# jewettaij/visfd

Measured on AMD Instinct MI355X. Metric: Mvoxels/s (Gauss+DoG+TV pipeline) on 1024^3 float32; % HBM roofline, higher is better.
Workload: dtype f32

## Files before the change

visfd_amd/csrc/blob.hip:

```cpp
#include <algorithm>
#include <cstdlib>
#include <limits>

#include "common.hpp"

namespace vh {

namespace {

constexpr int BLOCK = 512;
constexpr int TX = 64, TY = 8;
constexpr int PZ = 4;
constexpr int BUFCAP = 2 * PZ * BLOCK;
constexpr int LW = TX + 2, LH = TY + 2;

static_assert(BLOCK == 512 && TX == 64, "candidate codes pack the thread index in 9 bits");

struct Cand {
  int ix, iy, iz;
  int kind;
  float score;
};

__global__ void __launch_bounds__(BLOCK)
blob_candidates_kernel(const float* __restrict__ mid, const float* __restrict__ mask, int nx, int ny, int nz,
                       float min_thr, float max_thr, int zchunk, int tiles_x, int tiles_y,
                       unsigned long long* __restrict__ out, unsigned long long capacity,
                       unsigned long long* __restrict__ counter) {
  constexpr int NLD = (LH * LW + BLOCK - 1) / BLOCK;
  __shared__ float tile[PZ][NLD * BLOCK];
  __shared__ unsigned int buf[BUFCAP];
  __shared__ unsigned int buf_n;
  __shared__ unsigned long long buf_base;
  if (threadIdx.x == 0) buf_n = 0;
  unsigned b = blockIdx.x;
  const int tile_x = b % tiles_x;
  b /= tiles_x;
  const int tile_y = b % tiles_y;
  const int chunk = b / tiles_y;
  const int x0 = tile_x * TX, y0 = tile_y * TY;
  const int zs = max(1, chunk * zchunk), ze = min(nz - 1, (chunk + 1) * zchunk);
  if (zs >= ze) return;
  const int tid = threadIdx.x;
  const int lx = tid & (TX - 1), ly = tid >> 6;
  const int gx = x0 + lx, gy = y0 + ly;
  const i64 plane = (i64)nx * ny;
  const bool interior = gx >= 1 && gx <= nx - 2 && gy >= 1 && gy <= ny - 2;

  unsigned ld_off[NLD];
#pragma unroll
  for (int k = 0; k < NLD; k++) {
    const int i = tid + k * BLOCK;
    const int r = i / LW, c = i - r * LW;
    const int sx = x0 - 1 + c, sy = y0 - 1 + r;
    ld_off[k] = (i < LH * LW && sx >= 0 && sx < nx && sy >= 0 && sy < ny) ? (unsigned)(sy * nx + sx) * 4u : 0x7ffffff0u;
  }
  const int plane_bytes = (int)(plane * 4);
  auto fetch = [&](int z, float v[NLD]) {
    const bool zin = z < nz;
    const __amdgpu_buffer_rsrc_t rs = __builtin_amdgcn_make_buffer_rsrc((void*)(mid + (zin ? (i64)z * plane : 0)), 0,
                                                                        zin ? plane_bytes : 0, 0x00020000);
#pragma unroll
    for (int k = 0; k < NLD; k++) v[k] = __builtin_bit_cast(float, __builtin_amdgcn_raw_buffer_load_b32(rs, (int)ld_off[k], 0, 0));
  };
  auto stash = [&](const float v[NLD], float* dst) {
#pragma unroll
    for (int k = 0; k < NLD; k++) dst[tid + k * BLOCK] = v[k];
  };
  auto minmax9 = [&](const float* t, float& mn, float& mx, float& centre) {
    const float* p0 = t + ly * LW + lx;
    float a = p0[0], bb = p0[1], c = p0[2];
    mn = fminf(fminf(a, bb), c); mx = fmaxf(fmaxf(a, bb), c);
    a = p0[LW]; bb = p0[LW + 1]; c = p0[LW + 2];
    centre = bb;
    mn = fminf(mn, fminf(fminf(a, bb), c)); mx = fmaxf(mx, fmaxf(fmaxf(a, bb), c));
    a = p0[2 * LW]; bb = p0[2 * LW + 1]; c = p0[2 * LW + 2];
    mn = fminf(mn, fminf(fminf(a, bb), c)); mx = fmaxf(mx, fmaxf(fmaxf(a, bb), c));
  };

  float mn_prev, mx_prev, c_prev, mn_cur, mx_cur, c_cur;
  float preA[PZ][NLD], preB[PZ][NLD];
  fetch(zs - 1, preA[0]);
  fetch(zs, preA[1]);
  stash(preA[0], tile[0]);
  stash(preA[1], tile[1]);
#pragma unroll
  for (int k = 0; k < PZ; k++) fetch(zs + 1 + k, preA[k]);
#pragma unroll
  for (int k = 0; k < PZ; k++) fetch(zs + PZ + 1 + k, preB[k]);
  __syncthreads();
  minmax9(tile[0], mn_prev, mx_prev, c_prev);
  minmax9(tile[1], mn_cur, mx_cur, c_cur);
  __syncthreads();
  auto step = [&](float (&pre)[PZ][NLD], int z0) {
#pragma unroll
    for (int k = 0; k < PZ; k++) stash(pre[k], tile[k]);
#pragma unroll
    for (int k = 0; k < PZ; k++) fetch(z0 + 2 * PZ + 1 + k, pre[k]);
    __syncthreads();
#pragma unroll
    for (int k = 0; k < PZ; k++) {
      const int z = z0 + k;
      if (z < ze) {
        float mn_nxt, mx_nxt, c_nxt;
        minmax9(tile[k], mn_nxt, mx_nxt, c_nxt);
        const float e = c_cur;
        const float bmin = fminf(fminf(mn_prev, mn_cur), mn_nxt);
        const float bmax = fmaxf(fmaxf(mx_prev, mx_cur), mx_nxt);
        const bool is_min = (e == bmin) && (e < 0.0f) && (e < min_thr);
        const bool is_max = (e == bmax) && (e > 0.0f) && (e > max_thr);
        {
          const i64 v = (i64)z * plane + (i64)gy * nx + gx;
          bool cand = interior && (is_min || is_max);
          if (cand && mask && mask[v] == 0.0f) cand = false;
          const unsigned long long bal = __ballot(cand);
          if (bal != 0ull) {
            const int lane = tid & 63;
            const int leader = __ffsll((long long)bal) - 1;
            unsigned int base = 0;
            if (lane == leader) base = atomicAdd(&buf_n, (unsigned int)__popcll(bal));
            base = (unsigned int)__shfl((int)base, leader);
            if (cand) buf[base + (unsigned int)__popcll(bal & ((1ull << lane) - 1ull))] = ((unsigned int)(z - zs) << 9) | (unsigned int)tid;
          }
        }
        mn_prev = mn_cur; mx_prev = mx_cur;
        mn_cur = mn_nxt; mx_cur = mx_nxt; c_cur = c_nxt;
      }
    }
    __syncthreads();
    const unsigned int n = buf_n;
    const bool last = z0 + PZ >= ze;
    if (n > (unsigned int)(BUFCAP - PZ * BLOCK) || (last && n)) {
      if (tid == 0) buf_base = atomicAdd(counter, (unsigned long long)n);
      __syncthreads();
      const unsigned long long base = buf_base;
      for (unsigned int i = tid; i < n; i += BLOCK)
        if (base + i < capacity) {
          const unsigned int code = buf[i];
          const int t = (int)(code & 511u), zz = zs + (int)(code >> 9);
          out[base + i] = (unsigned long long)((i64)zz * plane + (i64)(y0 + (t >> 6)) * nx + (x0 + (t & (TX - 1))));
        }
      __syncthreads();
      if (tid == 0) buf_n = 0;
    }
  };
  for (int z0 = zs; z0 < ze; z0 += 2 * PZ) {
    step(preA, z0);
    step(preB, z0 + PZ);
  }
}

__global__ void __launch_bounds__(BLOCK)
blob_verify_kernel(const unsigned long long* __restrict__ cand_idx, const unsigned long long* __restrict__ n_cand_ptr,
                   unsigned long long cand_capacity,
                   const float* __restrict__ lo, const float* __restrict__ mid, const float* __restrict__ hi,
                   const float* __restrict__ mask, int nx, int ny, int nz, float min_thr, float max_thr,
                   Cand* __restrict__ out, unsigned long long capacity, unsigned long long* __restrict__ counter) {
  unsigned long long n_cand = *n_cand_ptr;
  if (n_cand > cand_capacity) n_cand = cand_capacity;
  for (unsigned long long t = (unsigned long long)blockIdx.x * BLOCK + threadIdx.x; t < n_cand;
       t += (unsigned long long)gridDim.x * BLOCK) {
  const i64 c = (i64)cand_idx[t];
  const i64 plane = (i64)nx * ny;
  const int iz = (int)(c / plane);
  const int rem = (int)(c - (i64)iz * plane);
  const int iy = rem / nx, ix = rem - iy * nx;
  const float e = mid[c];
  bool is_min = (e < 0.0f) && (e < min_thr);
  bool is_max = (e > 0.0f) && (e > max_thr);
  {
    const float a = lo[c], b = hi[c];
    if (a <= e || b <= e) is_min = false;
    if (a >= e || b >= e) is_max = false;
  }
  const float* vol[3] = {mid, lo, hi};
  for (int r = 0; r < 3 && (is_min || is_max); r++) {
    const float* v = vol[r];
    for (int jz = -1; jz <= 1; jz++)
      for (int jy = -1; jy <= 1; jy++) {
        const i64 row = c + (i64)jz * plane + (i64)jy * nx;
#pragma unroll
        for (int jx = -1; jx <= 1; jx++) {
          if (r == 0 && jz == 0 && jy == 0 && jx == 0) continue;
          const i64 q = row + jx;
          if (mask && r == 0 && mask[q] == 0.0f) { is_min = false; is_max = false; }
          const float nb = v[q];
          if (nb <= e) is_min = false;
          if (nb >= e) is_max = false;
        }
      }
  }
  if (is_min || is_max) {
    const unsigned long long slot = atomicAdd(counter, 1ULL);
    if (slot < capacity) {
      Cand cd;
      cd.ix = ix; cd.iy = iy; cd.iz = iz;
      cd.kind = is_min ? 0 : 1;
      cd.score = e;
      out[slot] = cd;
    }
  }
  }
}

}

struct ScanBufs {
  unsigned long long* idx = nullptr;
  Cand* cand = nullptr;
  unsigned long long* counters = nullptr;
  size_t cap_idx = 0, cap_out = 0;
};

static int scan_bufs(visfd_hip_ctx* ctx, int set, ScanBufs* B, bool pipelined, i64 nvox) {
  constexpr size_t NSET = 3;
  size_t cap_idx = ctx->slot_bytes[WS_TVAUX] / sizeof(unsigned long long) / NSET;
  if (cap_idx < (1u << 22)) cap_idx = 1u << 22;
  if (cap_idx < (size_t)(nvox / 32)) cap_idx = (size_t)(nvox / 32);
  size_t cap_out = ctx->slot_bytes[WS_CAND] / sizeof(Cand) / NSET;
  if (cap_out < (1u << 20)) cap_out = 1u << 20;
  if (cap_out < (size_t)(nvox / 128)) cap_out = (size_t)(nvox / 128);
  unsigned long long* idx = nullptr;
  Cand* cand = nullptr;
  unsigned long long* counters = nullptr;
  VH_TRY(ws(ctx, WS_TVAUX, NSET * cap_idx, &idx));
  VH_TRY(ws(ctx, WS_CAND, NSET * cap_out, &cand));
  VH_TRY(ws(ctx, WS_SCANCNT, 8, &counters));
  B->idx = idx + (size_t)set * cap_idx;
  B->cand = cand + (size_t)set * cap_out;
  B->counters = counters + 2 * set;
  B->cap_idx = cap_idx;
  B->cap_out = cap_out;
  if (pipelined) {
    if (ctx->opt.blob_test_cap > 0) {
      const size_t v = (size_t)ctx->opt.blob_test_cap;
      if (v < B->cap_idx) B->cap_idx = v;
      if (v < B->cap_out) B->cap_out = v;
    }
  }
  return VISFD_HIP_OK;
}

static void sort_and_append(std::vector<Cand>& h, i64 nx, i64 ny, int scale_index, float sigma,
                            std::vector<visfd_hip_blob>* minima, std::vector<visfd_hip_blob>* maxima) {
  const size_t m = h.size();
  std::vector<unsigned long long> key(m), key2(m);
  std::vector<unsigned int> pos(m), pos2(m);
  unsigned long long maxkey = 0;
  for (size_t i = 0; i < m; i++) {
    key[i] = (unsigned long long)(((i64)h[i].iz * ny + h[i].iy) * nx + h[i].ix);
    pos[i] = (unsigned int)i;
    if (key[i] > maxkey) maxkey = key[i];
  }
  constexpr int RB = 11;
  for (int shift = 0; shift < 64 && (maxkey >> shift) != 0; shift += RB) {
    size_t hist[(1 << RB) + 1] = {0};
    for (size_t i = 0; i < m; i++) hist[((key[i] >> shift) & ((1u << RB) - 1)) + 1]++;
    for (int b = 0; b < (1 << RB); b++) hist[b + 1] += hist[b];
    for (size_t i = 0; i < m; i++) {
      const size_t d = hist[(key[i] >> shift) & ((1u << RB) - 1)]++;
      key2[d] = key[i];
      pos2[d] = pos[i];
    }
    key.swap(key2);
    pos.swap(pos2);
  }
  for (size_t i = 0; i < m; i++) {
    const Cand& cd = h[pos[i]];
    visfd_hip_blob bl;
    bl.ix = cd.ix; bl.iy = cd.iy; bl.iz = cd.iz;
    bl.scale = scale_index;
    bl.sigma = sigma;
    bl.score = cd.score;
    (cd.kind == 0 ? minima : maxima)->push_back(bl);
  }
}

static int scan_enqueue(visfd_hip_ctx* ctx, const ScanBufs& B, const float* lo, const float* mid, const float* hi,
                        const float* mask, i64 nx, i64 ny, i64 nz, float min_thr, float max_thr) {
  hipStream_t st = ctx->stream;
  if (nx * ny >= (1LL << 29)) return fail(VISFD_HIP_EINVAL, "planes of 2 GiB and more are not supported by the blob scan");
  const int tiles_x = (int)((nx + TX - 1) / TX), tiles_y = (int)((ny + TY - 1) / TY);
  const i64 tiles = (i64)tiles_x * tiles_y;
  i64 want_chunks = ((i64)ctx->num_cus * 16 + tiles - 1) / tiles;
  if (want_chunks < 1) want_chunks = 1;
  i64 zchunk = (nz + want_chunks - 1) / want_chunks;
  if (zchunk < 16) zchunk = 16;
  const i64 nchunks = (nz + zchunk - 1) / zchunk;
  const i64 nblocks = tiles * nchunks;
  if (nblocks > 0x7fffffffLL) return fail(VISFD_HIP_EINVAL, "volume too large for one launch");
  VH_HIP(hipMemsetAsync(B.counters, 0, 2 * sizeof(unsigned long long), st));
  blob_candidates_kernel<<<dim3((unsigned)nblocks), dim3(BLOCK), 0, st>>>(
      mid, mask, (int)nx, (int)ny, (int)nz, min_thr, max_thr, (int)zchunk, tiles_x, tiles_y, B.idx,
      (unsigned long long)B.cap_idx, B.counters);
  VH_HIP(hipGetLastError());
  blob_verify_kernel<<<dim3((unsigned)(ctx->num_cus * 8)), dim3(BLOCK), 0, st>>>(
      B.idx, B.counters, (unsigned long long)B.cap_idx, lo, mid, hi, mask, (int)nx, (int)ny, (int)nz, min_thr, max_thr,
      B.cand, (unsigned long long)B.cap_out, B.counters + 1);
  VH_HIP(hipGetLastError());
  return VISFD_HIP_OK;
}

int blob_scan_launch(visfd_hip_ctx* ctx, const BlobJob* owner, int set, hipEvent_t done, const float* lo, const float* mid,
                     const float* hi, const float* mask, i64 nx, i64 ny, i64 nz, float min_thr, float max_thr,
                     ScanPending* pending) {
  VH_TRY(blob_jobs_drain(ctx, owner));
  ScanBufs B;
  VH_TRY(scan_bufs(ctx, set, &B, true, nx * ny * nz));
  VH_TRY(scan_enqueue(ctx, B, lo, mid, hi, mask, nx, ny, nz, min_thr, max_thr));
  VH_HIP(hipEventRecord(done, ctx->stream));
  pending->counters = B.counters;
  pending->survivors = B.cand;
  pending->cap_idx = B.cap_idx;
  pending->cap_out = B.cap_out;
  return VISFD_HIP_OK;
}

int blob_scan_collect(visfd_hip_ctx* ctx, const ScanPending& B, hipEvent_t done, hipStream_t aux, i64 nx, i64 ny,
                      int scale_index,
                      float sigma, std::vector<visfd_hip_blob>* minima, std::vector<visfd_hip_blob>* maxima,
                      bool* overflow) {
  *overflow = false;
  VH_HIP(hipStreamWaitEvent(aux, done, 0));
  unsigned long long c2[2] = {0, 0};
  VH_HIP(hipMemcpyAsync(c2, B.counters, sizeof(c2), hipMemcpyDeviceToHost, aux));
  VH_HIP(hipStreamSynchronize(aux));
  if (ctx->opt.debug) fprintf(stderr, "[blob scan] scale %d: %llu candidates, %llu blobs\n", scale_index, c2[0], c2[1]);
  if (c2[0] > B.cap_idx || c2[1] > B.cap_out) { *overflow = true; return VISFD_HIP_OK; }
  std::vector<Cand> h((size_t)c2[1]);
  if (c2[1]) {
    VH_HIP(hipMemcpyAsync(h.data(), B.survivors, sizeof(Cand) * (size_t)c2[1], hipMemcpyDeviceToHost, aux));
    VH_HIP(hipStreamSynchronize(aux));
  }
  sort_and_append(h, nx, ny, scale_index, sigma, minima, maxima);
  return VISFD_HIP_OK;
}

int dev_blob_scan(visfd_hip_ctx* ctx, const float* lo, const float* mid, const float* hi,
                  const float* mask, i64 nx, i64 ny, i64 nz, int scale_index, float sigma,
                  float min_thr, float max_thr, bool want_min, bool want_max,
                  std::vector<visfd_hip_blob>* minima, std::vector<visfd_hip_blob>* maxima) {
  if (nx < 3 || ny < 3 || nz < 3) return VISFD_HIP_OK;
  if (nx >= (1LL << 31) || ny >= (1LL << 31) || nz >= (1LL << 31))
    return fail(VISFD_HIP_EINVAL, "dimension too large");
  const float inf = std::numeric_limits<float>::infinity();
  if (!want_min) min_thr = -inf;
  if (!want_max) max_thr = inf;
  hipStream_t st = ctx->stream;
  VH_TRY(blob_jobs_drain(ctx));
  for (int attempt = 0; attempt < 4; attempt++) {
    ScanBufs B;
    VH_TRY(scan_bufs(ctx, 0, &B, false, nx * ny * nz));
    VH_TRY(scan_enqueue(ctx, B, lo, mid, hi, mask, nx, ny, nz, min_thr, max_thr));
    unsigned long long c2[2] = {0, 0};
    VH_HIP(hipMemcpyAsync(c2, B.counters, sizeof(c2), hipMemcpyDeviceToHost, st));
    VH_HIP(hipStreamSynchronize(st));
    if (ctx->opt.debug) fprintf(stderr, "[blob scan] scale %d: %llu candidates\n", scale_index, c2[0]);
    if (c2[0] > B.cap_idx) {
      unsigned long long* p = nullptr;
      VH_TRY(ws(ctx, WS_TVAUX, 3 * (size_t)c2[0] + 16, &p));
      continue;
    }
    if (c2[1] > B.cap_out) {
      Cand* p = nullptr;
      VH_TRY(ws(ctx, WS_CAND, 3 * (size_t)c2[1] + 16, &p));
      continue;
    }
    std::vector<Cand> h((size_t)c2[1]);
    if (c2[1]) {
      VH_HIP(hipMemcpyAsync(h.data(), B.cand, sizeof(Cand) * (size_t)c2[1], hipMemcpyDeviceToHost, st));
      VH_HIP(hipStreamSynchronize(st));
    }
    sort_and_append(h, nx, ny, scale_index, sigma, minima, maxima);
    return VISFD_HIP_OK;
  }
  return fail(VISFD_HIP_EDEVICE, "blob candidate list kept overflowing");
}

}
```

visfd_amd/csrc/gauss_pair.hip:

```cpp
#include <type_traits>

#include "common.hpp"

namespace vh {

namespace {

constexpr int Z_NT = 256;
constexpr int Z_PF = 8;
constexpr int YX_NT = 256;
constexpr int YX_PF = 12;
constexpr int Z_CHUNK = 256;
constexpr int Y_CHUNK = 512;

template <int H>
struct PairTaps {
  float a[H + 1], b[H + 1];
};

template <int B, int E, class F>
__device__ __forceinline__ void static_for(F&& f) {
  if constexpr (B < E) {
    f(std::integral_constant<int, B>{});
    static_for<B + 1, E>(f);
  }
}

template <int H>
__device__ __forceinline__ void taps_to_vgprs(const PairTaps<H>& tp, float (&ta)[H + 1], float (&tb)[H + 1]) {
#pragma unroll
  for (int m = 0; m <= H; m++) {
    ta[m] = tp.a[m];
    tb[m] = tp.b[m];
    asm volatile("" : "+v"(ta[m]));
    asm volatile("" : "+v"(tb[m]));
  }
}

template <int H, int U>
__device__ __forceinline__ void scatter(float (&ring)[2 * H + 1], const float (&t)[H + 1], float x) {
  constexpr int W = 2 * H + 1;
  float pr[H + 1];
#pragma unroll
  for (int m = 0; m <= H; m++) pr[m] = t[m] * x;
#pragma unroll
  for (int j = -H; j <= H; j++) {
    const int s = (U + H - j) % W;
    if (j == -H) ring[s] = pr[H];
    else ring[s] = ring[s] + pr[j < 0 ? -j : j];
    asm volatile("" : "+v"(ring[s]));
  }
}

template <int H>
__global__ void __launch_bounds__(Z_NT, 4)
pair_z_kernel(const float* __restrict__ src, float* __restrict__ za, float* __restrict__ zb, PairTaps<H> tp, i64 plane, int nz,
              int zchunk) {
  constexpr int W = 2 * H + 1;
  const i64 c = (i64)blockIdx.x * Z_NT + threadIdx.x;
  if (c >= plane) return;
  float ta[H + 1], tb[H + 1];
  taps_to_vgprs<H>(tp, ta, tb);
  const int zs = blockIdx.y * zchunk;
  const int ze = min(zs + zchunk, nz);
  const int nsteps = ze - zs + 2 * H;
  const int ktop = ze - 1 + H;
  const float* p = src + c;
  auto load = [&](int s) -> float { return p[(i64)min(max(ktop - s, 0), nz - 1) * plane]; };
  auto inside = [&](int s) -> bool { return ktop - s >= 0 && ktop - s < nz; };
  float ra[W], rb[W], q[Z_PF];
#pragma unroll
  for (int m = 0; m < W; m++) ra[m] = rb[m] = 0.0f;
#pragma unroll
  for (int i = 0; i < Z_PF; i++) q[i] = load(i);
#pragma nounroll
  for (int nb = 0; nb < nsteps; nb += W) {
    static_for<0, W>([&](auto U) {
      constexpr int u = decltype(U)::value;
      const int s = nb + u;
      const float x = inside(s) ? q[0] : 0.0f;
#pragma unroll
      for (int i = 0; i + 1 < Z_PF; i++) q[i] = q[i + 1];
      q[Z_PF - 1] = load(s + Z_PF);
      scatter<H, u>(ra, ta, x);
      scatter<H, u>(rb, tb, x);
      const int z = ktop + H - s;
      const bool done = s >= 2 * H && z >= zs;
      const i64 o = done ? (i64)z * plane : 0;
      const int len = done ? (int)(plane * 4) : 0;
      const __amdgpu_buffer_rsrc_t sa = __builtin_amdgcn_make_buffer_rsrc((void*)(za + o), 0, len, 0x00020000);
      const __amdgpu_buffer_rsrc_t sb = __builtin_amdgcn_make_buffer_rsrc((void*)(zb + o), 0, len, 0x00020000);
      __builtin_amdgcn_raw_buffer_store_b32(__builtin_bit_cast(unsigned, ra[u]), sa, (int)c * 4, 0, 2);
      __builtin_amdgcn_raw_buffer_store_b32(__builtin_bit_cast(unsigned, rb[u]), sb, (int)c * 4, 0, 2);
      __builtin_amdgcn_sched_barrier(0);
    });
  }
}

template <int H>
struct YxCfg {
  static constexpr int W = 2 * H + 1;
  static constexpr int XW = (2 * H + 4 + 3) / 4;
  static constexpr int TX = YX_NT + 4 - 4 * XW;
  static constexpr int QPR = TX / 4;
  static constexpr int LDS = (int)sizeof(float) * (2 * W * YX_NT + 2 * TX + 2 * Y_CHUNK);
  static_assert(TX % 4 == 0 && TX + 2 * H <= YX_NT && TX > 0, "tile width");
  static_assert(LDS <= 64 * 1024, "LDS rows of both filters and the normaliser lines");
  static_assert(H > 8 || 4 * LDS <= 160 * 1024, "four workgroups per CU up to H = 8");
};

template <int H>
__global__ void __launch_bounds__(YX_NT, 3)
pair_yx_kernel(const float* __restrict__ za, const float* __restrict__ zb, float* __restrict__ dst, PairTaps<H> tp,
               const float* __restrict__ Da, const float* __restrict__ Db, i64 dz_offset, int nx, int ny, int ychunk,
               int xtiles, int ychunks, float scale, int vec_ok) {
  typedef YxCfg<H> C;
  constexpr int W = C::W;
  __shared__ __attribute__((aligned(16))) float sA[W][YX_NT];
  __shared__ __attribute__((aligned(16))) float sB[W][YX_NT];
  __shared__ __attribute__((aligned(16))) float sKx[2][C::TX];
  __shared__ float sKy[2][Y_CHUNK];
  float ta[H + 1], tb[H + 1];
  taps_to_vgprs<H>(tp, ta, tb);
  unsigned b = blockIdx.x;
  const int bx = b % xtiles;
  b /= xtiles;
  const int by = b % ychunks;
  const int z = b / ychunks;
  const int tid = threadIdx.x;
  const int x0 = bx * C::TX;
  const int xc = x0 - H + tid;
  const bool col_ok = xc >= 0 && xc < nx;
  const bool idle = x0 - H + 64 * __builtin_amdgcn_readfirstlane(tid >> 6) >= nx;
  const int ys = by * ychunk;
  const int ye = min(ys + ychunk, ny);
  const int nsteps = ye - ys + 2 * H;
  const int ktop = ye - 1 + H;
  const i64 zoff = (i64)z * nx * ny;
  const float* pa = za + zoff + min(max(xc, 0), nx - 1);
  const float* pb = zb + zoff + min(max(xc, 0), nx - 1);
  auto row_off = [&](int s) -> i64 { return (i64)min(max(ktop - s, 0), ny - 1) * nx; };
  auto inside = [&](int s) -> bool { return col_ok && ktop - s >= 0 && ktop - s < ny; };
  float ra[W], rb[W], qa[YX_PF], qb[YX_PF];
#pragma unroll
  for (int m = 0; m < W; m++) ra[m] = rb[m] = 0.0f;
  if (!idle) {
#pragma unroll
    for (int i = 0; i < YX_PF; i++) {
      qa[i] = pa[row_off(i)];
      qb[i] = pb[row_off(i)];
    }
  } else {
#pragma unroll
    for (int i = 0; i < YX_PF; i++) qa[i] = qb[i] = 0.0f;
#pragma unroll
    for (int m = 0; m < W; m++) sA[m][tid] = sB[m][tid] = 0.0f;
  }
  const float* Dax = Da; const float* Day = Da + nx; const float* Daz = Da + nx + ny + dz_offset;
  const float* Dbx = Db; const float* Dby = Db + nx; const float* Dbz = Db + nx + ny + dz_offset;
  const float daz = Daz[z], dbz = Dbz[z];
  if (tid < C::TX) {
    const int xi = min(x0 + tid, nx - 1);
    sKx[0][tid] = Dax[xi];
    sKx[1][tid] = Dbx[xi];
  }
  for (int i = tid; i < ye - ys; i += YX_NT) {
    sKy[0][i] = Day[ys + i];
    sKy[1][i] = Dby[ys + i];
  }
  float* const out_plane = dst + zoff;
  const int QV = min(C::QPR, (nx - x0 + 3) >> 2);
  const int u_first = tid / QV, q_first = tid - u_first * QV;
  const int u_step = YX_NT / QV, q_step = YX_NT - u_step * QV;

  auto x_task = [&](int u, int qd, int nb) {
    const int s = nb + u;
    const int y = ktop + H - s;
    const int x = x0 + 4 * qd;
    if (s < 2 * H || y < ys || x >= nx) return;
    float ga[4], gb[4];
    {
      float v[4 * C::XW];
#pragma unroll
      for (int k = 0; k < C::XW; k++) {
        const float4 t4 = *reinterpret_cast<const float4*>(&sA[u][4 * qd + 4 * k]);
        v[4 * k] = t4.x; v[4 * k + 1] = t4.y; v[4 * k + 2] = t4.z; v[4 * k + 3] = t4.w;
      }
#pragma unroll
      for (int jj = 0; jj < W; jj++) {
        const float t = ta[jj < H ? H - jj : jj - H];
#pragma unroll
        for (int k = 0; k < 4; k++) {
          const float term = t * v[2 * H - jj + k];
          ga[k] = jj == 0 ? term : ga[k] + term;
        }
      }
    }
    {
      float v[4 * C::XW];
#pragma unroll
      for (int k = 0; k < C::XW; k++) {
        const float4 t4 = *reinterpret_cast<const float4*>(&sB[u][4 * qd + 4 * k]);
        v[4 * k] = t4.x; v[4 * k + 1] = t4.y; v[4 * k + 2] = t4.z; v[4 * k + 3] = t4.w;
      }
#pragma unroll
      for (int jj = 0; jj < W; jj++) {
        const float t = tb[jj < H ? H - jj : jj - H];
#pragma unroll
        for (int k = 0; k < 4; k++) {
          const float term = t * v[2 * H - jj + k];
          gb[k] = jj == 0 ? term : gb[k] + term;
        }
      }
    }
    const float4 ka = *reinterpret_cast<const float4*>(&sKx[0][4 * qd]);
    const float4 kb = *reinterpret_cast<const float4*>(&sKx[1][4 * qd]);
    const float dxa[4] = {ka.x, ka.y, ka.z, ka.w}, dxb[4] = {kb.x, kb.y, kb.z, kb.w};
    const float day = sKy[0][y - ys], dby = sKy[1][y - ys];
    float da[4], db[4];
    bool ones = true;
#pragma unroll
    for (int k = 0; k < 4; k++) {
      ga[k] = ga[k] + 0.0f;
      gb[k] = gb[k] + 0.0f;
      da[k] = (dxa[k] * day) * daz;
      db[k] = (dxb[k] * dby) * dbz;
      ones = ones && da[k] == 1.0f && db[k] == 1.0f;
    }
    if (__builtin_amdgcn_ballot_w64(!ones) != 0ull) {
#pragma unroll
      for (int k = 0; k < 4; k++) {
        ga[k] = ga[k] / da[k];
        gb[k] = gb[k] / db[k];
      }
    }
    float r[4];
#pragma unroll
    for (int k = 0; k < 4; k++) {
      const float dd = ga[k] - gb[k];
      r[k] = dd * scale;
    }
    float* o = out_plane + (i64)y * nx + x;
    if (vec_ok && x + 3 < nx) {
      typedef float v4f __attribute__((ext_vector_type(4)));
      const v4f r4 = {r[0], r[1], r[2], r[3]};
      __builtin_nontemporal_store(r4, reinterpret_cast<v4f*>(o));
    } else {
#pragma unroll
      for (int k = 0; k < 4; k++)
        if (x + k < nx) __builtin_nontemporal_store(r[k], &o[k]);
    }
  };
  auto march_step = [&](auto U, int nb) {
    constexpr int u = decltype(U)::value;
    const int s = nb + u;
    const bool in = inside(s);
    const float xa = in ? qa[0] : 0.0f, xb = in ? qb[0] : 0.0f;
#pragma unroll
    for (int i = 0; i + 1 < YX_PF; i++) { qa[i] = qa[i + 1]; qb[i] = qb[i + 1]; }
    qa[YX_PF - 1] = pa[row_off(s + YX_PF)];
    qb[YX_PF - 1] = pb[row_off(s + YX_PF)];
    scatter<H, u>(ra, ta, xa);
    scatter<H, u>(rb, tb, xb);
    sA[u][tid] = ra[u];
    sB[u][tid] = rb[u];
    __builtin_amdgcn_sched_barrier(0);
  };

#pragma nounroll
  for (int nb = 0; nb < nsteps; nb += W) {
    if (!idle) static_for<0, W>([&](auto U) { march_step(U, nb); });
    __syncthreads();
    for (int u = u_first, qd = q_first; u < W;) {
      x_task(u, qd, nb);
      u += u_step;
      qd += q_step;
      if (qd >= QV) { qd -= QV; u++; }
    }
    __syncthreads();
  }
}

constexpr int PAIR_H_MIN = 6, PAIR_H_MAX = 10;
const bool kPairWins[PAIR_H_MAX + 1] = {false, false, false, false, false, false,  true,  true,  true,
                                         true,  true};

bool bit_symmetric(const Taps& T) {
  for (int j = 1; j <= T.h; j++)
    if (std::memcmp(&T.t[T.h + j], &T.t[T.h - j], sizeof(float)) != 0) return false;
  return true;
}
bool same_bits(const Taps& A, const Taps& B) {
  return A.h == B.h && std::memcmp(A.t, B.t, sizeof(float) * (2 * A.h + 1)) == 0;
}

template <int H>
int launch_pair(visfd_hip_ctx* ctx, const LogPairRequest& rq, const float* Da, const float* Db) {
  typedef YxCfg<H> C;
  const i64 nx = rq.nx, ny = rq.ny, nz = rq.nz, plane = nx * ny, n = plane * nz;
  float *za = nullptr, *zb = nullptr;
  VH_TRY(ws(ctx, WS_A, (size_t)n, &za));
  VH_TRY(ws(ctx, WS_B, (size_t)n, &zb));
  PairTaps<H> tz, tyx;
  for (int m = 0; m <= H; m++) {
    tz.a[m] = rq.a[2].t[H + m];  tz.b[m] = rq.b[2].t[H + m];
    tyx.a[m] = rq.a[0].t[H + m]; tyx.b[m] = rq.b[0].t[H + m];
  }
  const int opt_chunk = ctx->opt.log_pair_chunk;
  i64 zchunk = opt_chunk > 0 ? opt_chunk : Z_CHUNK;
  if ((nz + zchunk - 1) / zchunk > 65535) zchunk = (nz + 65534) / 65535;
  const i64 zblocks = (plane + Z_NT - 1) / Z_NT, zchunks = (nz + zchunk - 1) / zchunk;
  const i64 ychunk = opt_chunk > 0 && opt_chunk < Y_CHUNK ? opt_chunk : Y_CHUNK;
  const i64 xtiles = (nx + C::TX - 1) / C::TX, ychunks = (ny + ychunk - 1) / ychunk;
  const i64 yxblocks = xtiles * ychunks * nz;
  if (zblocks > 0x7fffffffLL || yxblocks > 0x7fffffffLL) return fail(VISFD_HIP_EINVAL, "volume too large for one launch");
  pair_z_kernel<H><<<dim3((unsigned)zblocks, (unsigned)zchunks), dim3(Z_NT), 0, ctx->stream>>>(rq.src, za, zb, tz, plane, (int)nz,
                                                                                                (int)zchunk);
  VH_HIP(hipGetLastError());
  const int vec_ok = ((nx & 3) == 0) && ((reinterpret_cast<uintptr_t>(rq.dst) & 15) == 0);
  pair_yx_kernel<H><<<dim3((unsigned)yxblocks), dim3(YX_NT), 0, ctx->stream>>>(za, zb, rq.dst, tyx, Da, Db, rq.z_lo, (int)nx, (int)ny,
                                                                                (int)ychunk, (int)xtiles, (int)ychunks, rq.scale,
                                                                                vec_ok);
  VH_HIP(hipGetLastError());
  return VISFD_HIP_OK;
}

}

int log_pair_route(visfd_hip_ctx* ctx, const LogPairRequest& rq) {
  const int mode = ctx->opt.log_pair;
  const int H = rq.a[0].h;
  if (mode == 0 || ctx->opt.gauss_3pass || H < PAIR_H_MIN || H > PAIR_H_MAX) return GAUSS_DECLINED;
  if (mode == 1 && !kPairWins[H]) return GAUSS_DECLINED;
  if (rq.nx <= 0 || rq.ny <= 0 || rq.nz <= 0 || rq.nx * rq.ny >= (1LL << 29) || rq.nz >= (1LL << 31)) return GAUSS_DECLINED;
  for (int d = 0; d < 3; d++)
    if (rq.a[d].h != H || rq.b[d].h != H || !bit_symmetric(rq.a[d]) || !bit_symmetric(rq.b[d])) return GAUSS_DECLINED;
  if (!same_bits(rq.a[0], rq.a[1]) || !same_bits(rq.b[0], rq.b[1])) return GAUSS_DECLINED;
  const i64 nz_global = rq.nz_global ? rq.nz_global : rq.nz;
  const i64 lines = rq.nx + rq.ny + nz_global;
  float* D = nullptr;
  VH_TRY(ws(ctx, WS_NORM, (size_t)(2 * lines), &D));
  VH_TRY(dev_norm_lines(ctx, D, rq.nx, rq.ny, nz_global, rq.a[0], rq.a[1], rq.a[2]));
  VH_TRY(dev_norm_lines(ctx, D + lines, rq.nx, rq.ny, nz_global, rq.b[0], rq.b[1], rq.b[2]));
  switch (H) {
    case 6: return launch_pair<6>(ctx, rq, D, D + lines);
    case 7: return launch_pair<7>(ctx, rq, D, D + lines);
    case 8: return launch_pair<8>(ctx, rq, D, D + lines);
    case 9: return launch_pair<9>(ctx, rq, D, D + lines);
    default: return launch_pair<10>(ctx, rq, D, D + lines);
  }
}

}
```

Before: 2589.

## Rewrite blob scan as per-wave register column marcher with DPP neighbors

The blob candidate kernel drops the shared-memory plane tiles and block-wide barriers. Each wave now marches along z over a 62-column by 4-row strip held in registers, with a 3-plane ring of prefetched rows. It takes x-neighbour min/max through DPP lane shifts and appends candidates to a per-wave buffer that it flushes with its own atomic. The gauss pair kernel splits the divide-by-normalisation ballot into separate a/b checks and raises wave priority during the X tasks. Optional timestamp probes are added to both kernels. The overlapping strips (62 useful columns of 64) load some data twice, and register pressure rises under the new occupancy hint.

```diff
diff --git a/visfd_amd/csrc/blob.hip b/visfd_amd/csrc/blob.hip
--- a/visfd_amd/csrc/blob.hip
+++ b/visfd_amd/csrc/blob.hip
@@ -1,6 +1,7 @@
 #include <algorithm>
 #include <cstdlib>
 #include <limits>
+#include <type_traits>
 
 #include "common.hpp"
 
@@ -9,12 +10,19 @@
 namespace {
 
 constexpr int BLOCK = 512;
-constexpr int TX = 64, TY = 8;
-constexpr int PZ = 4;
-constexpr int BUFCAP = 2 * PZ * BLOCK;
-constexpr int LW = TX + 2, LH = TY + 2;
-
-static_assert(BLOCK == 512 && TX == 64, "candidate codes pack the thread index in 9 bits");
+constexpr int SWV = BLOCK / 64;
+constexpr int SOX = 62;
+constexpr int SR = 4;
+constexpr int SPF = 3;
+constexpr int WCAP = 2 * SR * 64;
+static_assert(SPF % 3 == 0, "the plane ring is indexed statically");
+
+#ifdef VH_BLOB_STAMPS
+__device__ unsigned long long g_blob_stamps[8];
+#define VH_STAMP(i) do { const unsigned long long t_ = __builtin_amdgcn_s_memtime(); st_acc[i] += t_ - st_last; st_last = t_; } while (0)
+#else
+#define VH_STAMP(i) do { } while (0)
+#endif
 
 struct Cand {
   int ix, iy, iz;
@@ -22,132 +30,146 @@
   float score;
 };
 
-__global__ void __launch_bounds__(BLOCK)
+template <int B, int E, class F>
+__device__ __forceinline__ void static_for(F&& f) {
+  if constexpr (B < E) {
+    f(std::integral_constant<int, B>{});
+    static_for<B + 1, E>(f);
+  }
+}
+
+__device__ __forceinline__ float lane_below(float v) {
+  return __builtin_bit_cast(float, __builtin_amdgcn_mov_dpp(__builtin_bit_cast(int, v), 0x138, 0xf, 0xf, true));
+}
+__device__ __forceinline__ float lane_above(float v) {
+  return __builtin_bit_cast(float, __builtin_amdgcn_mov_dpp(__builtin_bit_cast(int, v), 0x130, 0xf, 0xf, true));
+}
+
+__global__ void __launch_bounds__(BLOCK, 6)
 blob_candidates_kernel(const float* __restrict__ mid, const float* __restrict__ mask, int nx, int ny, int nz,
                        float min_thr, float max_thr, int zchunk, int tiles_x, int tiles_y,
                        unsigned long long* __restrict__ out, unsigned long long capacity,
                        unsigned long long* __restrict__ counter) {
-  constexpr int NLD = (LH * LW + BLOCK - 1) / BLOCK;
-  __shared__ float tile[PZ][NLD * BLOCK];
-  __shared__ unsigned int buf[BUFCAP];
-  __shared__ unsigned int buf_n;
-  __shared__ unsigned long long buf_base;
-  if (threadIdx.x == 0) buf_n = 0;
+  __shared__ unsigned long long buf[SWV][WCAP];
   unsigned b = blockIdx.x;
   const int tile_x = b % tiles_x;
   b /= tiles_x;
   const int tile_y = b % tiles_y;
   const int chunk = b / tiles_y;
-  const int x0 = tile_x * TX, y0 = tile_y * TY;
   const int zs = max(1, chunk * zchunk), ze = min(nz - 1, (chunk + 1) * zchunk);
   if (zs >= ze) return;
-  const int tid = threadIdx.x;
-  const int lx = tid & (TX - 1), ly = tid >> 6;
-  const int gx = x0 + lx, gy = y0 + ly;
+  const int lane = threadIdx.x & 63;
+  const int wave = __builtin_amdgcn_readfirstlane(threadIdx.x >> 6);
+  const int gx = tile_x * SOX + lane;
+  const int yb = tile_y * (SWV * SR) + wave * SR;
+  if (yb + 1 > ny - 2) return;
+#ifdef VH_BLOB_STAMPS
+  unsigned long long st_acc[4] = {0, 0, 0, 0};
+  unsigned long long st_last = __builtin_amdgcn_s_memtime();
+#endif
   const i64 plane = (i64)nx * ny;
-  const bool interior = gx >= 1 && gx <= nx - 2 && gy >= 1 && gy <= ny - 2;
-
-  unsigned ld_off[NLD];
-#pragma unroll
-  for (int k = 0; k < NLD; k++) {
-    const int i = tid + k * BLOCK;
-    const int r = i / LW, c = i - r * LW;
-    const int sx = x0 - 1 + c, sy = y0 - 1 + r;
-    ld_off[k] = (i < LH * LW && sx >= 0 && sx < nx && sy >= 0 && sy < ny) ? (unsigned)(sy * nx + sx) * 4u : 0x7ffffff0u;
-  }
+  const bool col_ok = lane >= 1 && lane <= SOX && gx <= nx - 2;
+  unsigned long long* const wbuf = buf[wave];
+
+  const int col_off = min(gx, nx - 1) * 4;
+  int row_off[SR + 2];
+#pragma unroll
+  for (int r = 0; r < SR + 2; r++) row_off[r] = min(yb + r, ny - 1) * nx * 4;
   const int plane_bytes = (int)(plane * 4);
-  auto fetch = [&](int z, float v[NLD]) {
-    const bool zin = z < nz;
-    const __amdgpu_buffer_rsrc_t rs = __builtin_amdgcn_make_buffer_rsrc((void*)(mid + (zin ? (i64)z * plane : 0)), 0,
-                                                                        zin ? plane_bytes : 0, 0x00020000);
-#pragma unroll
-    for (int k = 0; k < NLD; k++) v[k] = __builtin_bit_cast(float, __builtin_amdgcn_raw_buffer_load_b32(rs, (int)ld_off[k], 0, 0));
+  auto fetch = [&](int z, float (&v)[SR + 2]) {
+    const __amdgpu_buffer_rsrc_t rs = __builtin_amdgcn_make_buffer_rsrc((void*)(mid + (i64)min(z, ze) * plane), 0, plane_bytes,
+                                                                        0x00020000);
+#pragma unroll
+    for (int r = 0; r < SR + 2; r++) v[r] = __builtin_bit_cast(float, __builtin_amdgcn_raw_buffer_load_b32(rs, col_off, row_off[r], 0));
   };
-  auto stash = [&](const float v[NLD], float* dst) {
-#pragma unroll
-    for (int k = 0; k < NLD; k++) dst[tid + k * BLOCK] = v[k];
+  const int p0 = (yb + 1) * nx + gx;
+  unsigned cnt = 0;
+  auto flush = [&]() {
+    unsigned long long base = 0;
+    if (lane == 0) base = atomicAdd(counter, (unsigned long long)cnt);
+    base = __shfl(base, 0);
+    __builtin_amdgcn_fence(__ATOMIC_RELEASE, "wavefront");
+    __builtin_amdgcn_wave_barrier();
+    __builtin_amdgcn_fence(__ATOMIC_ACQUIRE, "wavefront");
+    for (unsigned i = lane; i < cnt; i += 64)
+      if (base + i < capacity) out[base + i] = wbuf[i];
+    __builtin_amdgcn_fence(__ATOMIC_RELEASE, "wavefront");
+    __builtin_amdgcn_wave_barrier();
+    cnt = 0;
   };
-  auto minmax9 = [&](const float* t, float& mn, float& mx, float& centre) {
-    const float* p0 = t + ly * LW + lx;
-    float a = p0[0], bb = p0[1], c = p0[2];
-    mn = fminf(fminf(a, bb), c); mx = fmaxf(fmaxf(a, bb), c);
-    a = p0[LW]; bb = p0[LW + 1]; c = p0[LW + 2];
-    centre = bb;
-    mn = fminf(mn, fminf(fminf(a, bb), c)); mx = fmaxf(mx, fmaxf(fmaxf(a, bb), c));
-    a = p0[2 * LW]; bb = p0[2 * LW + 1]; c = p0[2 * LW + 2];
-    mn = fminf(mn, fminf(fminf(a, bb), c)); mx = fmaxf(mx, fmaxf(fmaxf(a, bb), c));
-  };
-
-  float mn_prev, mx_prev, c_prev, mn_cur, mx_cur, c_cur;
-  float preA[PZ][NLD], preB[PZ][NLD];
-  fetch(zs - 1, preA[0]);
-  fetch(zs, preA[1]);
-  stash(preA[0], tile[0]);
-  stash(preA[1], tile[1]);
-#pragma unroll
-  for (int k = 0; k < PZ; k++) fetch(zs + 1 + k, preA[k]);
-#pragma unroll
-  for (int k = 0; k < PZ; k++) fetch(zs + PZ + 1 + k, preB[k]);
-  __syncthreads();
-  minmax9(tile[0], mn_prev, mx_prev, c_prev);
-  minmax9(tile[1], mn_cur, mx_cur, c_cur);
-  __syncthreads();
-  auto step = [&](float (&pre)[PZ][NLD], int z0) {
-#pragma unroll
-    for (int k = 0; k < PZ; k++) stash(pre[k], tile[k]);
-#pragma unroll
-    for (int k = 0; k < PZ; k++) fetch(z0 + 2 * PZ + 1 + k, pre[k]);
-    __syncthreads();
-#pragma unroll
-    for (int k = 0; k < PZ; k++) {
-      const int z = z0 + k;
-      if (z < ze) {
-        float mn_nxt, mx_nxt, c_nxt;
-        minmax9(tile[k], mn_nxt, mx_nxt, c_nxt);
-        const float e = c_cur;
-        const float bmin = fminf(fminf(mn_prev, mn_cur), mn_nxt);
-        const float bmax = fmaxf(fmaxf(mx_prev, mx_cur), mx_nxt);
-        const bool is_min = (e == bmin) && (e < 0.0f) && (e < min_thr);
-        const bool is_max = (e == bmax) && (e > 0.0f) && (e > max_thr);
-        {
-          const i64 v = (i64)z * plane + (i64)gy * nx + gx;
-          bool cand = interior && (is_min || is_max);
+
+  float m9n[3][SR], m9x[3][SR], ctr[3][SR];
+#pragma unroll
+  for (int k = 0; k < 3; k++)
+#pragma unroll
+    for (int j = 0; j < SR; j++) m9n[k][j] = m9x[k][j] = ctr[k][j] = 0.0f;
+  float q[SPF][SR + 2];
+#pragma unroll
+  for (int i = 0; i < SPF; i++) {
+    fetch(zs - 1 + i, q[i]);
+    __builtin_amdgcn_sched_barrier(0);
+  }
+  const int nsteps = ze - zs + 2;
+  VH_STAMP(0);
+#pragma nounroll
+  for (int nb = 0; nb < nsteps; nb += SPF) {
+    static_for<0, SPF>([&](auto U) {
+      constexpr int u = decltype(U)::value;
+      constexpr int nxt = u % 3, cur = (u + 2) % 3, prv = (u + 1) % 3;
+      const int t = nb + u;
+      float hn[SR + 2], hx[SR + 2], hc[SR + 2];
+#pragma unroll
+      for (int r = 0; r < SR + 2; r++) {
+        const float v = q[u][r], lo = lane_below(v), hi = lane_above(v);
+        hn[r] = fminf(fminf(lo, v), hi);
+        hx[r] = fmaxf(fmaxf(lo, v), hi);
+        hc[r] = v;
+      }
+      __builtin_amdgcn_sched_barrier(0);
+      fetch(zs - 1 + t + SPF, q[u]);
+      __builtin_amdgcn_sched_barrier(0);
+#pragma unroll
+      for (int j = 0; j < SR; j++) {
+        m9n[nxt][j] = fminf(fminf(hn[j], hn[j + 1]), hn[j + 2]);
+        m9x[nxt][j] = fmaxf(fmaxf(hx[j], hx[j + 1]), hx[j + 2]);
+        asm volatile("v_mov_b32 %0, %1" : "=v"(ctr[nxt][j]) : "v"(hc[j + 1]));
+      }
+      VH_STAMP(1);
+      const int z = zs + t - 2;
+      if (t >= 2 && z < ze) {
+#pragma unroll
+        for (int j = 0; j < SR; j++) {
+          const int gy = yb + 1 + j;
+          const float e = ctr[cur][j];
+          const float bmin = fminf(fminf(m9n[prv][j], m9n[cur][j]), m9n[nxt][j]);
+          const float bmax = fmaxf(fmaxf(m9x[prv][j], m9x[cur][j]), m9x[nxt][j]);
+          const bool is_min = (e == bmin) && (e < 0.0f) && (e < min_thr);
+          const bool is_max = (e == bmax) && (e > 0.0f) && (e > max_thr);
+          const i64 v = (i64)z * plane + (p0 + j * nx);
+          bool cand = col_ok && gy <= ny - 2 && (is_min || is_max);
           if (cand && mask && mask[v] == 0.0f) cand = false;
           const unsigned long long bal = __ballot(cand);
           if (bal != 0ull) {
-            const int lane = tid & 63;
-            const int leader = __ffsll((long long)bal) - 1;
-            unsigned int base = 0;
-            if (lane == leader) base = atomicAdd(&buf_n, (unsigned int)__popcll(bal));
-            base = (unsigned int)__shfl((int)base, leader);
-            if (cand) buf[base + (unsigned int)__popcll(bal & ((1ull << lane) - 1ull))] = ((unsigned int)(z - zs) << 9) | (unsigned int)tid;
+            if (cand) wbuf[cnt + (unsigned)__popcll(bal & ((1ull << lane) - 1ull))] = (unsigned long long)v;
+            cnt += (unsigned)__popcll(bal);
           }
         }
-        mn_prev = mn_cur; mx_prev = mx_cur;
-        mn_cur = mn_nxt; mx_cur = mx_nxt; c_cur = c_nxt;
+        VH_STAMP(2);
+        if (cnt > (unsigned)(WCAP - SR * 64)) {
+          flush();
+          VH_STAMP(3);
+        }
       }
-    }
-    __syncthreads();
-    const unsigned int n = buf_n;
-    const bool last = z0 + PZ >= ze;
-    if (n > (unsigned int)(BUFCAP - PZ * BLOCK) || (last && n)) {
-      if (tid == 0) buf_base = atomicAdd(counter, (unsigned long long)n);
-      __syncthreads();
-      const unsigned long long base = buf_base;
-      for (unsigned int i = tid; i < n; i += BLOCK)
-        if (base + i < capacity) {
-          const unsigned int code = buf[i];
-          const int t = (int)(code & 511u), zz = zs + (int)(code >> 9);
-          out[base + i] = (unsigned long long)((i64)zz * plane + (i64)(y0 + (t >> 6)) * nx + (x0 + (t & (TX - 1))));
-        }
-      __syncthreads();
-      if (tid == 0) buf_n = 0;
-    }
-  };
-  for (int z0 = zs; z0 < ze; z0 += 2 * PZ) {
-    step(preA, z0);
-    step(preB, z0 + PZ);
-  }
+    });
+  }
+  if (cnt) flush();
+  VH_STAMP(3);
+#ifdef VH_BLOB_STAMPS
+  if (lane == 0) {
+#pragma unroll
+    for (int i = 0; i < 4; i++) atomicAdd(&g_blob_stamps[i], st_acc[i]);
+  }
+#endif
 }
 
 __global__ void __launch_bounds__(BLOCK)
@@ -280,7 +302,8 @@
                         const float* mask, i64 nx, i64 ny, i64 nz, float min_thr, float max_thr) {
   hipStream_t st = ctx->stream;
   if (nx * ny >= (1LL << 29)) return fail(VISFD_HIP_EINVAL, "planes of 2 GiB and more are not supported by the blob scan");
-  const int tiles_x = (int)((nx + TX - 1) / TX), tiles_y = (int)((ny + TY - 1) / TY);
+  const int tiles_x = (int)std::max<i64>(1, (nx - 2 + SOX - 1) / SOX);
+  const int tiles_y = (int)std::max<i64>(1, (ny - 2 + SWV * SR - 1) / (SWV * SR));
   const i64 tiles = (i64)tiles_x * tiles_y;
   i64 want_chunks = ((i64)ctx->num_cus * 16 + tiles - 1) / tiles;
   if (want_chunks < 1) want_chunks = 1;
@@ -298,6 +321,18 @@
       B.idx, B.counters, (unsigned long long)B.cap_idx, lo, mid, hi, mask, (int)nx, (int)ny, (int)nz, min_thr, max_thr,
       B.cand, (unsigned long long)B.cap_out, B.counters + 1);
   VH_HIP(hipGetLastError());
+#ifdef VH_BLOB_STAMPS
+  {
+    unsigned long long st8[8], z8[8] = {};
+    VH_HIP(hipStreamSynchronize(st));
+    VH_HIP(hipMemcpyFromSymbol(st8, HIP_SYMBOL(g_blob_stamps), sizeof(st8)));
+    double tot = 0;
+    for (int i = 0; i < 4; i++) tot += (double)st8[i];
+    fprintf(stderr, "[blob scan stamps] share of wave time: prologue %.3f | wait for the plane + row and 3x3 extrema + requests %.3f | "
+            "tests + append %.3f | flush %.3f  (total %.4g ticks)\n", st8[0] / tot, st8[1] / tot, st8[2] / tot, st8[3] / tot, tot);
+    VH_HIP(hipMemcpyToSymbol(HIP_SYMBOL(g_blob_stamps), z8, sizeof(z8)));
+  }
+#endif
   return VISFD_HIP_OK;
 }
 
diff --git a/visfd_amd/csrc/gauss_pair.hip b/visfd_amd/csrc/gauss_pair.hip
--- a/visfd_amd/csrc/gauss_pair.hip
+++ b/visfd_amd/csrc/gauss_pair.hip
@@ -12,6 +12,13 @@
 constexpr int YX_PF = 12;
 constexpr int Z_CHUNK = 256;
 constexpr int Y_CHUNK = 512;
+
+#ifdef VH_PAIR_STAMPS
+__device__ unsigned long long g_pair_stamps[8];
+#define VH_STAMP(i) do { const unsigned long long t_ = __builtin_amdgcn_s_memtime(); st_acc[i] += t_ - st_last; st_last = t_; } while (0)
+#else
+#define VH_STAMP(i) do { } while (0)
+#endif
 
 template <int H>
 struct PairTaps {
@@ -120,6 +127,10 @@
   __shared__ __attribute__((aligned(16))) float sB[W][YX_NT];
   __shared__ __attribute__((aligned(16))) float sKx[2][C::TX];
   __shared__ float sKy[2][Y_CHUNK];
+#ifdef VH_PAIR_STAMPS
+  unsigned long long st_acc[5] = {0, 0, 0, 0, 0};
+  unsigned long long st_last = __builtin_amdgcn_s_memtime();
+#endif
   float ta[H + 1], tb[H + 1];
   taps_to_vgprs<H>(tp, ta, tb);
   unsigned b = blockIdx.x;
@@ -218,21 +229,23 @@
     const float dxa[4] = {ka.x, ka.y, ka.z, ka.w}, dxb[4] = {kb.x, kb.y, kb.z, kb.w};
     const float day = sKy[0][y - ys], dby = sKy[1][y - ys];
     float da[4], db[4];
-    bool ones = true;
+    bool ones_a = true, ones_b = true;
 #pragma unroll
     for (int k = 0; k < 4; k++) {
       ga[k] = ga[k] + 0.0f;
       gb[k] = gb[k] + 0.0f;
       da[k] = (dxa[k] * day) * daz;
       db[k] = (dxb[k] * dby) * dbz;
-      ones = ones && da[k] == 1.0f && db[k] == 1.0f;
-    }
-    if (__builtin_amdgcn_ballot_w64(!ones) != 0ull) {
-#pragma unroll
-      for (int k = 0; k < 4; k++) {
-        ga[k] = ga[k] / da[k];
-        gb[k] = gb[k] / db[k];
-      }
+      ones_a = ones_a && da[k] == 1.0f;
+      ones_b = ones_b && db[k] == 1.0f;
+    }
+    if (__builtin_amdgcn_ballot_w64(!ones_a) != 0ull) {
+#pragma unroll
+      for (int k = 0; k < 4; k++) ga[k] = ga[k] / da[k];
+    }
+    if (__builtin_amdgcn_ballot_w64(!ones_b) != 0ull) {
+#pragma unroll
+      for (int k = 0; k < 4; k++) gb[k] = gb[k] / db[k];
     }
     float r[4];
 #pragma unroll
@@ -267,18 +280,31 @@
     __builtin_amdgcn_sched_barrier(0);
   };
 
+  VH_STAMP(0);
 #pragma nounroll
   for (int nb = 0; nb < nsteps; nb += W) {
     if (!idle) static_for<0, W>([&](auto U) { march_step(U, nb); });
+    VH_STAMP(1);
     __syncthreads();
+    VH_STAMP(2);
+    __builtin_amdgcn_s_setprio(2);
     for (int u = u_first, qd = q_first; u < W;) {
       x_task(u, qd, nb);
       u += u_step;
       qd += q_step;
       if (qd >= QV) { qd -= QV; u++; }
     }
+    __builtin_amdgcn_s_setprio(0);
+    VH_STAMP(3);
     __syncthreads();
-  }
+    VH_STAMP(4);
+  }
+#ifdef VH_PAIR_STAMPS
+  if ((tid & 63) == 0) {
+#pragma unroll
+    for (int i = 0; i < 5; i++) atomicAdd(&g_pair_stamps[i], st_acc[i]);
+  }
+#endif
 }
 
 constexpr int PAIR_H_MIN = 6, PAIR_H_MAX = 10;
@@ -322,6 +348,19 @@
                                                                                 (int)ychunk, (int)xtiles, (int)ychunks, rq.scale,
                                                                                 vec_ok);
   VH_HIP(hipGetLastError());
+#ifdef VH_PAIR_STAMPS
+  {
+    unsigned long long st8[8], z8[8] = {};
+    VH_HIP(hipStreamSynchronize(ctx->stream));
+    VH_HIP(hipMemcpyFromSymbol(st8, HIP_SYMBOL(g_pair_stamps), sizeof(st8)));
+    double tot = 0;
+    for (int i = 0; i < 5; i++) tot += (double)st8[i];
+    fprintf(stderr, "[pair_yx stamps H=%d] share of wave time: prologue %.3f | march %.3f | wait at barrier 1 %.3f | X tasks %.3f | "
+            "wait at barrier 2 %.3f  (total %.4g ticks over %lld waves)\n", H, st8[0] / tot, st8[1] / tot, st8[2] / tot, st8[3] / tot,
+            st8[4] / tot, tot, (long long)yxblocks * (YX_NT / 64));
+    VH_HIP(hipMemcpyToSymbol(HIP_SYMBOL(g_pair_stamps), z8, sizeof(z8)));
+  }
+#endif
   return VISFD_HIP_OK;
 }
 
```

Result: faster. 2624, median of 6 (+1.4%).
